# RazorClient/Stark-prover

Measured on AMD Instinct MI355X. Metric: FRI commit field-elems/sec at codeword 2^24; achieved HBM GB/s vs peak, higher is better.
Workload: dtype u32; 1 GPU; fri_commit codeword 2^24, blowup 8 (d=2^21), SHA-256 Merkle per layer, 21 rounds; codeword_log2=24, per_gpu_log2=24, blowup=8, field=p=3*2^30+1, parallelism=single GPU

## Files before the change

stark-prover_amd/csrc/fri_layer.hip:

```cpp
#include <cassert>
#include "fri_internal.hpp"
#include "sha256_fast.hpp"
#include "sha256_quad.hpp"

namespace fri {

#ifdef FRI_STAMPS
#define STAMP_WITH(on, i, fn)                                  \
    do {                                                       \
        if (on) t.st->stamps[t.k][(i)] = fn();                 \
    } while (0)
#else
#define STAMP_WITH(on, i, fn) do {} while (0)
#endif
#define STAMP(on, i) STAMP_WITH(on, i, __builtin_amdgcn_s_memrealtime)
#define STAMP_CLK(on, i) STAMP_WITH(on, i, __builtin_amdgcn_s_memtime)

#ifndef FRI_CHAIN_PRIO
#define FRI_CHAIN_PRIO 3
#endif
__device__ __forceinline__ void chain_prio() {
    if (FRI_CHAIN_PRIO > 0) __builtin_amdgcn_s_setprio(FRI_CHAIN_PRIO);
}

// ... 149 lines not shown
    coef_slice(t, w, G, red, 0, blockDim.x);
    lds_barrier();
    if (threadIdx.x == 0) coef_combine(t, w, red, blockDim.x / 64);
}

__device__ __forceinline__ void quad(const uint4& vals, uint32_t* lv0, uint32_t* lv1, size_t q ,
                                     Dg& out) {
    Dg a, b, c, d, n0, n1;
    hleaf(vals.x, a); hleaf(vals.y, b); hleaf(vals.z, c); hleaf(vals.w, d);
    dg_store(lv0 + 8 * (4 * q), a); dg_store(lv0 + 8 * (4 * q + 1), b);
    dg_store(lv0 + 8 * (4 * q + 2), c); dg_store(lv0 + 8 * (4 * q + 3), d);
    hnode(a, b, n0);
    hnode(c, d, n1);
    dg_store(lv1 + 8 * (2 * q), n0);
    dg_store(lv1 + 8 * (2 * q + 1), n1);
    hnode(n0, n1, out);
}

template <uint32_t TPB>
__device__ __forceinline__ void lds_two_levels(uint4* lds, const Dg& mine, uint32_t* lv2, uint32_t* lv3, uint32_t* lv4,
                                               size_t g2 ) {
    uint4* A = lds;
    uint4* B = lds + 2 * TPB;
    const uint32_t t = threadIdx.x;
    dg_store(lv2 + 8 * (g2 + t), mine);
    dg_lds_store(A + 2 * t, mine);
    lds_barrier();
    if (t < TPB / 2) {
        Dg l, r, o;
        dg_lds_load(A + 4 * t, l); dg_lds_load(A + 4 * t + 2, r);
        hnode(l, r, o);
        dg_lds_store(B + 2 * t, o);
        dg_store(lv3 + 8 * (g2 / 2 + t), o);
    }
    lds_barrier();
    if (t < TPB / 4) {
        Dg l, r, o;
        dg_lds_load(B + 4 * t, l); dg_lds_load(B + 4 * t + 2, r);
        hnode(l, r, o);
        dg_store(lv4 + 8 * (g2 / 4 + t), o);
    }
}

__device__ __forceinline__ bool gated_off(const LayerTask& t) {
    return t.gst && t.gidx >= 0 && !t.gst->active[t.gidx];
}

__device__ __forceinline__ uint32_t pair_beta(const LayerTask& t) { return t.gst->beta_mont[t.gidx]; }

template <bool FOLD, bool COMMIT, uint32_t TPB, bool PAIR = false>
__global__ __launch_bounds__(TPB) void k_layer_leaf(LayerTask t) {
    if (gated_off(t)) return;
    __shared__ uint4 lds[3 * TPB];
    __shared__ int32_t red[3 * (TPB / 64)];
    const uint32_t L = t.L;
    const size_t wg = PAIR ? (size_t)blockIdx.x + t.wg_base : (size_t)blockIdx.x;
    const size_t q = wg * TPB + threadIdx.x;
    uint4 v;
    if (FOLD) {
        const size_t half = (size_t)1 << L;
        const uint32_t beta_m = COMMIT ? t.st->beta_mont[t.k - 1] : (PAIR ? pair_beta(t) : t.beta_m);
        uint4 a = reinterpret_cast<const uint4*>(t.prev)[q];
        uint4 b = reinterpret_cast<const uint4*>(PAIR ? t.prev2 : t.prev + half)[q];
        uint4 x = reinterpret_cast<const uint4*>(t.xinv)[q];
        v.x = fold_one(a.x, b.x, x.x, beta_m); v.y = fold_one(a.y, b.y, x.y, beta_m);
        v.z = fold_one(a.z, b.z, x.z, beta_m); v.w = fold_one(a.w, b.w, x.w, beta_m);
        reinterpret_cast<uint4*>(t.values)[q] = v;
    } else {
        v = reinterpret_cast<const uint4*>(t.values)[q];
    }
    uint32_t* tr = t.tree;
    Dg top;
    quad(v, tr + 8 * level_offset(L, 0), tr + 8 * level_offset(L, 1), q, top);
    if (COMMIT) coef_task(t, blockIdx.x, gridDim.x, red);
    lds_two_levels<TPB>(lds, top, tr + 8 * level_offset(L, 2), tr + 8 * level_offset(L, 3),
                        tr + 8 * level_offset(L, 4), wg * TPB);
}

#ifndef WIDE_PAIR_MAX
#define WIDE_PAIR_MAX (1u << 16)
#endif

__host__ __device__ __forceinline__ uint32_t wide_levels(uint32_t L) { return L <= 8 + TOP_LOG ? 8u : 4u; }

template <bool FOLD, bool COMMIT, bool PAIR = false>
__global__ __launch_bounds__(256) void k_layer_leaf_wide(LayerTask t) {
    if (gated_off(t)) return;
    STAMP(COMMIT && blockIdx.x == 0 && threadIdx.x == 0, 60);
    __shared__ uint4 lds[2 * 256 + 2 * 128];
    __shared__ int32_t red[12];
    __shared__ SchedLds sl;
    sched_init(&sl);
    const uint32_t L = t.L;
    const size_t wg = PAIR ? (size_t)blockIdx.x + t.wg_base : (size_t)blockIdx.x;
    const size_t grid = PAIR ? (size_t)t.wg_total : (size_t)gridDim.x;
    const size_t i = wg * 256 + threadIdx.x;
    uint32_t v;
    if (FOLD) {
        const size_t half = (size_t)1 << L;
        const uint32_t beta_m = COMMIT ? t.st->beta_mont[t.k - 1] : (PAIR ? pair_beta(t) : t.beta_m);
        v = fold_one(t.prev[i], PAIR ? t.prev2[i] : t.prev[i + half], t.xinv[i], beta_m);
        t.values[i] = v;
    } else {
        v = t.values[i];
    }
    uint32_t* tr = t.tree;
    Dg d;
    cleaf(v, d);
    dg_store(tr + 8 * i, d);
    uint4* A = lds;
    uint4* B = lds + 2 * 256;
    dg_lds_store(A + 2 * threadIdx.x, d);
    lds_barrier();
    STAMP(COMMIT && blockIdx.x == 0 && threadIdx.x == 0, 61);
    uint32_t cnt = 256;
    const shaq::Role qr = shaq::role_of(threadIdx.x);
    if (grid * 128 < WIDE_PAIR_MAX) chain_prio();
    const uint32_t nlev = wide_levels(L);
#pragma unroll 1
    for (uint32_t j = 1; j <= nlev; j++) {
        cnt >>= 1;
        uint32_t* out = tr + 8 * (level_offset(L, j) + (wg << (8 - j)));
        if ((size_t)cnt * grid < WIDE_PAIR_MAX) {
            pair_level_s(A, B, out, threadIdx.x, cnt, qr, &sl, j);
        } else if (threadIdx.x < cnt) {
            Dg a, b, o;
            dg_lds_load(A + 4 * threadIdx.x, a);
            dg_lds_load(A + 4 * threadIdx.x + 2, b);
            hnode(a, b, o);
            dg_lds_store(B + 2 * threadIdx.x, o);
            dg_store(out + 8 * threadIdx.x, o);
        }
        if (COMMIT && j == 2 && threadIdx.x >= 128) coef_slice(t, blockIdx.x, gridDim.x, red, 128, 128);
        lds_barrier();
        uint4* tmp = A; A = B; B = tmp;
    }
    if (COMMIT && threadIdx.x == 128) coef_combine(t, blockIdx.x, red, 2);
    STAMP(COMMIT && blockIdx.x == 0 && threadIdx.x == 0, 62);
}

__device__ __forceinline__ void reduce_mx(const int32_t* in, int32_t* out, uint32_t w, uint32_t R) {
    if (threadIdx.x >= 64) return;
    Mx3 m;
    if (threadIdx.x < R) m.load(in, R * w + threadIdx.x);
    m.wave_max();
    if (threadIdx.x == 0) m.store(out, w);
}

__global__ __launch_bounds__(512) void k_tree_mid(uint32_t* tree, uint32_t L, uint32_t l, const DevState* st,
                                                  int gate, const int32_t* mx_in, int32_t* mx_out, uint32_t R) {
    if (st && gate >= 0 && !st->active[gate]) return;
    constexpr uint32_t NIN = 1024;
    __shared__ uint4 lds[NIN + NIN / 2];
    __shared__ SchedLds sl;
    sched_init(&sl);
    uint4* A = lds;
    uint4* B = lds + NIN;
    const uint32_t t = threadIdx.x;
    const size_t base = (size_t)blockIdx.x * NIN;
    const uint32_t* in = tree + 8 * level_offset(L, l);
    {
        Dg a, b, o;
        dg_load(in + 8 * (base + 2 * t), a);
        dg_load(in + 8 * (base + 2 * t + 1), b);
        if (mx_in) reduce_mx(mx_in, mx_out, blockIdx.x, R);
        hnode(a, b, o);
        dg_lds_store(A + 2 * t, o);
        dg_store(tree + 8 * (level_offset(L, l + 1) + (base >> 1) + t), o);
    }
    lds_barrier();
    const shaq::Role qr = shaq::role_of(t);
    uint32_t cnt = NIN / 2;
#pragma unroll 1
    for (uint32_t j = 2; j <= 4; j++) {
        cnt >>= 1;
        uint32_t* out = tree + 8 * (level_offset(L, l + j) + (base >> j));
        const bool narrow = (size_t)cnt * gridDim.x < WIDE_PAIR_MAX;
        if (narrow) {
            pair_level_s(A, B, out, t, cnt, qr, &sl, j);
        } else if (t < cnt) {
            Dg a, b, o;
            dg_lds_load(A + 4 * t, a);
            dg_lds_load(A + 4 * t + 2, b);
            hnode(a, b, o);
            dg_lds_store(B + 2 * t, o);
            dg_store(out + 8 * t, o);
        }
        lds_barrier();
        uint4* tmp = A; A = B; B = tmp;
    }
}

__global__ __launch_bounds__(256) void k_tree_mid8(uint32_t* tree, uint32_t L, uint32_t l, const DevState* st,
                                                   int gate, const int32_t* mx_in, int32_t* mx_out, uint32_t R) {
    if (st && gate >= 0 && !st->active[gate]) return;
    chain_prio();
    __shared__ uint4 lds[256 + 128];
    __shared__ SchedLds sl;
    sched_init(&sl);
    uint4* A = lds;
    uint4* B = lds + 256;
    const uint32_t t = threadIdx.x;
    const size_t base = (size_t)blockIdx.x * 256;
    const uint32_t* in = tree + 8 * level_offset(L, l);
    const shaq::Role qr = shaq::role_of(t);
    {
        const uint32_t q = t >> 1, half = (t & 1u) ^ 1u;
        Dg a, b;
        dg_load(in + 8 * (base + 2 * q), a);
        dg_load(in + 8 * (base + 2 * q + 1), b);
        if (mx_in) reduce_mx(mx_in, mx_out, blockIdx.x, R);
        uint32_t o[4];
        shaq::node(a.w, b.w, o, qr);
        const uint4 v = make_uint4(o[0], o[1], o[2], o[3]);
        A[2 * q + half] = v;
        reinterpret_cast<uint4*>(tree + 8 * (level_offset(L, l + 1) + (base >> 1) + q))[half] = v;
    }
    lds_barrier();
    uint32_t cnt = 128;
#pragma unroll 1
    for (uint32_t j = 2; j <= 8; j++) {
        cnt >>= 1;
        pair_level_s(A, B, tree + 8 * (level_offset(L, l + j) + (base >> j)), t, cnt, qr, &sl, j);
        lds_barrier();
        uint4* tmp = A; A = B; B = tmp;
    }
}

__device__ __forceinline__ void ktouch(const void* sym) {
    uint32_t a, b, c, d;
    asm volatile("s_nop 4\n\t"
                 "s_load_dword %0, %4, 0x0\n\ts_load_dword %1, %4, 0x40\n\t"
                 "s_load_dword %2, %4, 0x80\n\ts_load_dword %3, %4, 0xc0\n\t"
                 "s_waitcnt lgkmcnt(0)"
                 : "=&s"(a), "=&s"(b), "=&s"(c), "=&s"(d)
                 : "s"(sym)
                 : "memory");
}
__device__ __forceinline__ void kcache_touch_sha_tables() {
    ktouch(&shaf::KTAB[0]);
    ktouch(&shaf::PAD_KW_C.kw[0]);
    ktouch(&shaf::PAD_KW_1024.kw[0]);
    ktouch(&shaf::PAD_KW_1536.kw[0]);
}

__device__ __forceinline__ uint32_t hexch(uint32_t nib) { return nib < 10u ? 0x30u + nib : 0x57u + nib; }
__device__ __forceinline__ void hex2(uint32_t x, uint32_t& hi, uint32_t& lo) {
    hi = (hexch(x >> 28) << 24) | (hexch((x >> 24) & 15u) << 16) | (hexch((x >> 20) & 15u) << 8) | hexch((x >> 16) & 15u);
    lo = (hexch((x >> 12) & 15u) << 24) | (hexch((x >> 8) & 15u) << 16) | (hexch((x >> 4) & 15u) << 8) | hexch(x & 15u);
}
__device__ __forceinline__ uint32_t hexhex(uint32_t b) {
    const uint32_t x = ((b & 0xF0u) << 12) | (b & 0x0Fu);
    const uint32_t ge = ((x + 0x00060006u) >> 4) & 0x00010001u;
    return 0x33303330u + x + ge * 0x2F7u;
}

enum { CJ_REHASH = 0, CJ_MID = 2, CJ_ROOT = 3, CJ_FINAL = 6, CJ_END_ROUND = 6, CJ_END_FINAL = 8 };

__device__ __forceinline__ void chan_job(int j, uint32_t cs[8], uint32_t X[4], uint32_t has, const uint4* root_lds,
                                         uint32_t fv, const shaq::Role& R) {
    j = __builtin_amdgcn_readfirstlane(j);
    has = __builtin_amdgcn_readfirstlane(has);
    uint32_t w[16];
    const bool pad = (j == 1) || (j == 5);
    if (j == 0 || j == 2 || j == 6) {
#pragma unroll
        for (int i = 0; i < 8; i++) hex2(cs[i], w[2 * i], w[2 * i + 1]);
#pragma unroll
        for (int i = 0; i < 4; i++) X[i] = R.iv[i];
    } else if (j == 3 || j == 4) {
        const uint32_t b = (__lane_id() & 15u) + (j == 4 ? 16u : 0u);
        const uint32_t rw = reinterpret_cast<const uint32_t*>(root_lds)[b >> 2];
        const uint32_t hh = hexhex((rw >> (24 - 8 * (b & 3))) & 255u);
#pragma unroll
        for (int jj = 0; jj < 16; jj++) w[jj] = __builtin_amdgcn_readlane(hh, jj);
        if (j == 3 && !has) {
#pragma unroll
            for (int i = 0; i < 4; i++) X[i] = R.iv[i];
        }
    } else if (j == 7) {
#pragma unroll
        for (int i = 0; i < 16; i++) w[i] = 0u;
        w[0] = 0x30303030u; w[1] = 0x30303030u;
        hex2(fv, w[2], w[3]);
        w[4] = 0x80000000u;
        w[15] = 80u * 8u;
    }
    if (pad) shaq::compress_kw(X, j == 1 ? shaf::PAD_KW_C.kw : (has ? shaf::PAD_KW_1536.kw : shaf::PAD_KW_1024.kw), R);
    else shaq::compress(X, w, R);
    if (j == 1 || j == 5 || j == 7) {
#pragma unroll
        for (int i = 0; i < 4; i++) {
            const uint32_t o = shaq::swap01(X[i]);
            cs[i] = R.is_a ? X[i] : o;
            cs[4 + i] = R.is_a ? o : X[i];
        }
    }
}

constexpr uint32_t pow2_32k_mod_p(int k) {
    uint64_t r = 1;
    for (int j = 0; j < k; j++) r = (r << 32) % P;
    return (uint32_t)r;
}
__device__ __forceinline__ uint32_t chan_beta(const uint32_t s[8]) {
    constexpr uint32_t W[8] = {pow2_32k_mod_p(8), pow2_32k_mod_p(7), pow2_32k_mod_p(6), pow2_32k_mod_p(5),
                               pow2_32k_mod_p(4), pow2_32k_mod_p(3), pow2_32k_mod_p(2), pow2_32k_mod_p(1)};
    uint32_t t[8];
#pragma unroll
    for (int i = 0; i < 8; i++) t[i] = mmul(s[i] >= P ? s[i] - P : s[i], W[i]);
    return add(add(add(t[0], t[1]), add(t[2], t[3])), add(add(t[4], t[5]), add(t[6], t[7])));
}


template <typename Value>
__device__ __forceinline__ void leaf_loop(uint32_t N, uint32_t* tr, uint4* A, Value&& value) {
    for (uint32_t i = threadIdx.x; i < max(N, 64u); i += blockDim.x) {
        const uint32_t j = i & (N - 1);
        const bool real = i < N;
        const uint32_t v = value(j, real);
        Dg d;
        cleaf(v, d);
        if (real) {
            dg_store(tr + 8 * j, d);
            dg_lds_store(A + 2 * j, d);
        }
    }
}

__device__ __forceinline__ void level_step(const LayerTask& t, bool stamps, uint32_t it, const uint4* A, uint4* B,
                                           uint32_t* out, uint32_t cnt, const shaq::Role& R, SchedLds* sl,
                                           uint32_t ord) {
    const uint32_t tid = threadIdx.x;
    if (cnt <= 128) {
        STAMP_CLK(stamps && it < 18 && tid == 0, 24 + 2 * it);
        pair_level_s(A, B, out, tid, cnt, R, sl, ord);
        STAMP_CLK(stamps && it < 18 && tid == 0, 25 + 2 * it);
        return;
    }
#pragma unroll 1
    for (uint32_t q = tid; q < cnt; q += blockDim.x) {
        Dg a, b, o;
        dg_lds_load(A + 4 * q, a);
        dg_lds_load(A + 4 * q + 2, b);
#ifdef FRI_STAMPS
        if (stamps && it < 18 && q == 0) asm volatile("s_waitcnt lgkmcnt(0)" ::: "memory");
#endif
        STAMP_CLK(stamps && it < 18 && q == 0, 24 + 2 * it);
        cnode(a, b, o);
        STAMP_CLK(stamps && it < 18 && q == 0, 25 + 2 * it);
        dg_lds_store(B + 2 * q, o);
        dg_store(out + 8 * q, o);
    }
}

__device__ __forceinline__ int chan_drain(const LayerTask& t, int job, int job_end, bool level, uint32_t cnt,
                                           uint32_t cs[8], uint32_t X[4], uint32_t has, const uint4* root_lds,
                                           uint32_t fv, const shaq::Role& R) {
    if (job >= job_end || (level && !(cnt <= 192 && job < CJ_ROOT))) return job;
    do {
        STAMP(threadIdx.x == 448 && job == CJ_ROOT, 14);
        STAMP(threadIdx.x == 448 && job == CJ_ROOT + 2, 13);
        chan_job(job, cs, X, has, root_lds, fv, R);
        STAMP(threadIdx.x == 448 && job >= CJ_ROOT && job <= CJ_ROOT + 2, 20 + job - CJ_ROOT);
        job++;
    } while (!level && job < job_end);
    return job;
}

struct RoundOut { uint32_t active, beta_m; };
__device__ __forceinline__ RoundOut layer_results(const LayerTask& t, const Degree& dg, const uint32_t cs[8],
                                                  uint32_t fv, uint32_t fbeta1, const uint4* root_lds) {
    DevState* st = t.st;
    const int k = t.k, deg = dg.deg;
    if (dg.noncanon) {
        st->active[k] = 0;
// ... 231 lines not shown
                    const uint32_t c = t.coef_in[j];
                    if (c) m.m0 = max(m.m0, (int)j);
                    if (c >= P) m.m1 = 0;
                }
            } else {
                const uint32_t len = (uint32_t)(prev_deg + 1), nlen = (len + 1) / 2;
                const bool in_lds = li > 0 && k >= 2;
                for (uint32_t j = tx; j < nlen; j += nthr) {
                    const uint32_t e = in_lds ? prev_c[2 * j] : t.coef_in[2 * j];
                    const uint32_t o = (2 * j + 1 < len) ? (in_lds ? prev_c[2 * j + 1] : t.coef_in[2 * j + 1]) : 0u;
                    const uint32_t v = add(e, mmul(o, beta_m));
                    cur_c[j] = v;
                    if (v) m.m0 = (int)j;
                    if (e) m.m1 = (int)j;
                    if (o) m.m2 = (int)j;
                }
            }
            mx3_wave_to_red(m, red, tx);
        };
        if (!coef_late) coef_fold(0, blockDim.x);
        if (li == 0 && !coef_late) prefetch_x(0, blockDim.x);
        lds_barrier();
        STAMP(tid == 0, 1);
        STAMP_CLK(tid == 0, 17);
        Degree dg{1, false};
        int job_end = CJ_END_ROUND;
        uint32_t fv = 0;
        auto settle = [&](uint32_t nw) {
            dg = degree_of(k, mx3_from_red(red, nw));
            job_end = dg.deg < 1 ? CJ_END_FINAL : CJ_END_ROUND;
            if (chan_wave && dg.deg == 0) fv = (k == 0) ? t.coef_in[0] : cur_c[0];
        };
        if (!coef_late) settle(8);
        int job = CJ_END_FINAL;
        if (chan_wave) job = !has ? CJ_ROOT : (pending ? CJ_REHASH : CJ_MID);
        const uint32_t total = nlev + 1;
        uint32_t cnt = N;
#pragma unroll 1
        for (uint32_t it = 0; it < total; it++) {
            const bool level = it < nlev;
            if (level) {
                cnt >>= 1;
                level_step(t, true, it, A, B, tr + 8 * level_offset(L, 1 + it), cnt, R, &sl, ord++);
            }
            if (chan_wave) job = chan_drain(t, job, job_end, level, cnt, cs, X, has, A, fv, R);
            if (coef_late && it == coef_it && tid >= 256 && tid < 384) coef_fold(256, 128);
            if (li == 0 && coef_late && it == coef_it && tid >= 384 && tid < 448) prefetch_x(384, 64);
            lds_barrier();
            if (coef_late && it == coef_it) settle(2);
            if (level) {
                uint4* tmp = A; A = B; B = tmp;
                STAMP(tid == 0 && it < 11, 2 + it);
                STAMP_CLK(tid == 0 && it + 1 == nlev, 18);
                STAMP(tid == 0 && it + 1 == nlev, 19);
            }
        }
        if (tid == 448) {
            const RoundOut r = layer_results(t, dg, cs, fv, s_fbeta[li], A);
            s_beta_m = r.beta_m;
            s_active = r.active;
            s_deg = dg.deg;
        }
        if (chan_wave) { has = 1; pending = 1; }
        lds_barrier();
        if (!s_active) break;
        beta_m = s_beta_m;
        prev_deg = s_deg;
    }
}

static LayerTask with_gate(const LayerTask& in) {
    LayerTask t = in;
    if (t.st) { t.gst = t.st; t.gidx = t.k > 0 ? t.k - 1 : -1; }
    return t;
}

#ifndef QUAD_TPB
#define QUAD_TPB 512
#endif
#ifndef QUAD_MIN_LOG
#define QUAD_MIN_LOG 19
#endif

template <typename KernelLaunch>
static void pair_parts(LayerTask t, uint32_t G, hipStream_t s, const std::function<void()>& after_part1,
                       KernelLaunch&& go) {
    t.wg_total = G;
    if (!after_part1) {
        t.wg_base = 0;
        go(t, G);
        return;
    }
    const uint32_t h = G / 2;
    t.wg_base = t.send_half ? h : 0u;
    go(t, h);
    after_part1();
    t.wg_base = t.send_half ? 0u : h;
    go(t, h);
}

void launch_layer(const LayerTask& tin, hipStream_t s, hipEvent_t ev_leaf_end, const std::function<void()>& after_leaf,
                  hipEvent_t ev_before_top, const std::function<void()>& after_part1) {
    const LayerTask t = with_gate(tin);
    const uint32_t L = t.L;
    const bool fold = t.prev != nullptr;
    const bool commit = t.st != nullptr;
    const bool pair = t.prev2 != nullptr;
    const int32_t* nomx = nullptr;
    static_assert(TAIL_LOG == TOP_LOG, "every commit layer the top could take from its leaves goes to launch_tail");
    if (L <= TOP_LOG) {
        assert(!fold && !commit);
        hipLaunchKernelGGL((k_tree_top<true, false>), dim3(1), dim3(512), 0, s, t, 0u, nomx, 1u);
        if (ev_leaf_end) hipEventRecord(ev_leaf_end, s);
        return;
    }
    uint32_t G, out_per_wg;
    if (L >= QUAD_MIN_LOG) {
        constexpr uint32_t TPB = QUAD_TPB;
        G = (uint32_t)(((size_t)1 << L) / (4 * TPB));
        out_per_wg = TPB / 4;
        if (pair) {
            pair_parts(t, G, s, after_part1, [&](const LayerTask& tp, uint32_t g) {
                hipLaunchKernelGGL((k_layer_leaf<true, false, TPB, true>), dim3(g), dim3(TPB), 0, s, tp);
            });
        } else if (fold) {
            if (commit) hipLaunchKernelGGL((k_layer_leaf<true, true, TPB>), dim3(G), dim3(TPB), 0, s, t);
            else hipLaunchKernelGGL((k_layer_leaf<true, false, TPB>), dim3(G), dim3(TPB), 0, s, t);
        } else {
            if (commit) hipLaunchKernelGGL((k_layer_leaf<false, true, TPB>), dim3(G), dim3(TPB), 0, s, t);
            else hipLaunchKernelGGL((k_layer_leaf<false, false, TPB>), dim3(G), dim3(TPB), 0, s, t);
        }
    } else {
        G = 1u << (L - 8);
        out_per_wg = 256u >> wide_levels(L);
        if (pair) {
            pair_parts(t, G, s, after_part1, [&](const LayerTask& tp, uint32_t g) {
                hipLaunchKernelGGL((k_layer_leaf_wide<true, false, true>), dim3(g), dim3(256), 0, s, tp);
            });
        } else if (fold) {
            if (commit) hipLaunchKernelGGL((k_layer_leaf_wide<true, true>), dim3(G), dim3(256), 0, s, t);
            else hipLaunchKernelGGL((k_layer_leaf_wide<true, false>), dim3(G), dim3(256), 0, s, t);
        } else {
            if (commit) hipLaunchKernelGGL((k_layer_leaf_wide<false, true>), dim3(G), dim3(256), 0, s, t);
            else hipLaunchKernelGGL((k_layer_leaf_wide<false, false>), dim3(G), dim3(256), 0, s, t);
        }
    }
    if (ev_leaf_end) hipEventRecord(ev_leaf_end, s);
    if (after_leaf) after_leaf();
    const int gate = t.gidx;
    const int32_t* mx = commit ? t.wgmax : nullptr;
    size_t mx_off = 3 * (size_t)G;
    uint32_t l = L >= QUAD_MIN_LOG ? 4u : wide_levels(L);
    while (L - l > TOP_LOG) {
        const size_t nodes = (size_t)1 << (L - l);
        const bool eight = nodes < ((size_t)1 << 18);
        assert(!eight || L - l >= 8 + 6);
        const uint32_t nin = eight ? 256u : 1024u;
        const uint32_t grid = (uint32_t)(nodes / nin);
        const uint32_t R = nin / out_per_wg;
        int32_t* mx_out = commit ? t.wgmax + mx_off : nullptr;
        if (eight)
            hipLaunchKernelGGL(k_tree_mid8, dim3(grid), dim3(256), 0, s, t.tree, L, l, t.gst, gate, mx, mx_out, R);
        else
            hipLaunchKernelGGL(k_tree_mid, dim3(grid), dim3(512), 0, s, t.tree, L, l, t.gst, gate, mx, mx_out, R);
        if (commit) { mx = mx_out; mx_off += 3 * (size_t)grid; }
        G = grid;
        out_per_wg = eight ? 1u : nin / 16;
        l += eight ? 8u : 4u;
    }
    if (ev_before_top) hipStreamWaitEvent(s, ev_before_top, 0);
    if (commit) hipLaunchKernelGGL((k_tree_top<false, true>), dim3(1), dim3(512), 0, s, t, l, mx, G);
    else if (t.shard) hipLaunchKernelGGL((k_tree_top<false, false, true>), dim3(1), dim3(512), 0, s, t, l, nomx, G);
    else hipLaunchKernelGGL((k_tree_top<false, false>), dim3(1), dim3(512), 0, s, t, l, nomx, G);
}

void launch_tail(const LayerTask* ts, uint32_t n, hipStream_t s) {
    TailTask tt{};
    tt.n = n;
    for (uint32_t i = 0; i < n; i++) tt.t[i] = ts[i];
    tt.t[0] = with_gate(ts[0]);
    if (ts[0].prev) hipLaunchKernelGGL((k_tree_tail<true>), dim3(1), dim3(512), 0, s, tt);
    else hipLaunchKernelGGL((k_tree_tail<false>), dim3(1), dim3(512), 0, s, tt);
}

__global__ __launch_bounds__(256) void k_coef(LayerTask t) {
    if (gated_off(t)) return;
    __shared__ int32_t red[12];
    coef_task(t, blockIdx.x, gridDim.x, red);
}

void launch_coef(const LayerTask& tin, uint32_t G, hipStream_t s) {
    const LayerTask t = with_gate(tin);
    hipLaunchKernelGGL(k_coef, dim3(G), dim3(256), 0, s, t);
}

void launch_top(const LayerTask& tin, uint32_t l, const int32_t* mx, uint32_t G, hipStream_t s) {
    const LayerTask t = with_gate(tin);
    if (t.shard) hipLaunchKernelGGL((k_tree_top<false, true, true>), dim3(1), dim3(512), 0, s, t, l, mx, G);
    else hipLaunchKernelGGL((k_tree_top<false, true>), dim3(1), dim3(512), 0, s, t, l, mx, G);
}

}
```

stark-prover_amd/csrc/sha256_quad.hpp:

```cpp
#pragma once
#include <stdint.h>
#include "sha256_fast.hpp"

namespace fri {
namespace shaq {

constexpr int SWAP01 = 1 | (0 << 2) | (3 << 4) | (2 << 6);

__device__ __forceinline__ uint32_t swap01(uint32_t v) {
    return (uint32_t)__builtin_amdgcn_update_dpp(0, (int)v, SWAP01, 0xF, 0xF, true);
}
__device__ __forceinline__ uint32_t rot(uint32_t x, uint32_t n) { return __builtin_amdgcn_alignbit(x, x, n); }
#define bop(a, b, c, tt) __builtin_amdgcn_bitop3_b32((a), (b), (c), (tt))

struct Role {
    uint32_t r1, r2, r3;
    uint32_t m;
    uint32_t me;
    uint32_t q1, q2, q3;
    uint32_t is_a;
    uint32_t iv[4];
};

__device__ __forceinline__ Role role_of(uint32_t lane) {
    Role r{};
    const uint32_t IV[8] = {0x6a09e667u, 0xbb67ae85u, 0x3c6ef372u, 0xa54ff53au,
                            0x510e527fu, 0x9b05688cu, 0x1f83d9abu, 0x5be0cd19u};
    if ((lane & 1u) == 0) {
        r.r1 = 6; r.r2 = 11; r.r3 = 25; r.m = 0u; r.me = ~0u;
        r.q1 = 17; r.q2 = 19; r.q3 = 10; r.is_a = 0u;
        for (int i = 0; i < 4; i++) r.iv[i] = IV[4 + i];
    } else {
        r.r1 = 2; r.r2 = 13; r.r3 = 22; r.m = ~0u; r.me = 0u;
        r.q1 = 7; r.q2 = 18; r.q3 = 3; r.is_a = ~0u;
        for (int i = 0; i < 4; i++) r.iv[i] = IV[i];
    }
    return r;
}

#define SHAQ_R(kw)                                                                   \
    {                                                                                \
        const uint32_t _S = bop(rot(x0, R.r1), rot(x0, R.r2), rot(x0, R.r3), 0x96);  \
        const uint32_t _sel = bop(x0, x1, R.m, 0x2D);        \
        const uint32_t _F = bop(_sel, x2, x1, 0xCA);              \
        const uint32_t _hk = (x3 + (kw)) & R.me;                                     \
        const uint32_t _V = _S + _F + _hk;                                           \
        const uint32_t _Z = bop(R.me, _V, x3, 0xCA);                \
        const uint32_t _n = _V + swap01(_Z);                                         \
        x3 = x2; x2 = x1; x1 = x0; x0 = _n;                                          \
    }

#define SHAQ_W(i)                                                                            \
    {                                                                                        \
        const uint32_t _x = bop(R.is_a, w[((i) + 1) & 15], w[((i) + 14) & 15], 0xCA);        \
        const uint32_t _s = bop(rot(_x, R.q1), rot(_x, R.q2), _x >> R.q3, 0x96);             \
        w[i] = w[i] + w[((i) + 9) & 15] + _s + swap01(_s);                                   \
    }

__device__ __forceinline__ void compress(uint32_t st[4], uint32_t w[16], const Role& R) {
    uint32_t x0 = st[0], x1 = st[1], x2 = st[2], x3 = st[3];
#pragma unroll
    for (int i = 0; i < 16; i++) SHAQ_R(w[i] + shaf::KTAB[i]);
#pragma unroll 1
    for (int r = 1; r < 4; r++) {
#pragma unroll
        for (int i = 0; i < 16; i++) {
            SHAQ_W(i);
            SHAQ_R(w[i] + shaf::KTAB[16 * r + i]);
        }
    }
    st[0] += x0; st[1] += x1; st[2] += x2; st[3] += x3;
}
__device__ __forceinline__ void compress_kw(uint32_t st[4], const uint32_t* kw, const Role& R) {
    uint32_t x0 = st[0], x1 = st[1], x2 = st[2], x3 = st[3];
#pragma unroll 1
    for (int r = 0; r < 4; r++) {
#pragma unroll
        for (int i = 0; i < 16; i++) SHAQ_R(kw[16 * r + i]);
    }
    st[0] += x0; st[1] += x1; st[2] += x2; st[3] += x3;
}
__device__ __forceinline__ void produce(uint32_t w[16], uint32_t* wk, uint32_t* flag, uint32_t base, bool store,
                                        bool flag_lane, const Role& R) {
#pragma unroll 1
    for (int b = 0; b < 3; b++) {
#pragma unroll
        for (int i = 0; i < 16; i++) SHAQ_W(i);
        if (store) {
            uint4* o = reinterpret_cast<uint4*>(wk + 16 * b);
#pragma unroll
            for (int j = 0; j < 4; j++)
                o[j] = make_uint4(w[4 * j] + shaf::KTAB[16 * (b + 1) + 4 * j],
                                  w[4 * j + 1] + shaf::KTAB[16 * (b + 1) + 4 * j + 1],
                                  w[4 * j + 2] + shaf::KTAB[16 * (b + 1) + 4 * j + 2],
                                  w[4 * j + 3] + shaf::KTAB[16 * (b + 1) + 4 * j + 3]);
        }
        if (flag_lane) __hip_atomic_store(flag, base + b + 1, __ATOMIC_RELEASE, __HIP_MEMORY_SCOPE_WORKGROUP);
    }
}

__device__ __forceinline__ void node_ext(const uint32_t l[8], const uint32_t r[8], uint32_t out[4], const Role& R,
                                         const uint32_t* wk, const uint32_t* flag, uint32_t base) {
    uint32_t x0 = R.iv[0], x1 = R.iv[1], x2 = R.iv[2], x3 = R.iv[3];
#pragma unroll
    for (int i = 0; i < 8; i++) SHAQ_R(l[i] + shaf::KTAB[i]);
#pragma unroll
    for (int i = 0; i < 8; i++) SHAQ_R(r[i] + shaf::KTAB[8 + i]);
#pragma unroll 1
    for (int b = 0; b < 3; b++) {
        while (__hip_atomic_load(flag, __ATOMIC_ACQUIRE, __HIP_MEMORY_SCOPE_WORKGROUP) < base + b + 1) {}
        const uint4* q = reinterpret_cast<const uint4*>(wk + 16 * b);
        const uint4 q0 = q[0], q1 = q[1], q2 = q[2], q3 = q[3];
        SHAQ_R(q0.x); SHAQ_R(q0.y); SHAQ_R(q0.z); SHAQ_R(q0.w);
        SHAQ_R(q1.x); SHAQ_R(q1.y); SHAQ_R(q1.z); SHAQ_R(q1.w);
        SHAQ_R(q2.x); SHAQ_R(q2.y); SHAQ_R(q2.z); SHAQ_R(q2.w);
        SHAQ_R(q3.x); SHAQ_R(q3.y); SHAQ_R(q3.z); SHAQ_R(q3.w);
    }
    out[0] = R.iv[0] + x0; out[1] = R.iv[1] + x1; out[2] = R.iv[2] + x2; out[3] = R.iv[3] + x3;
    compress_kw(out, shaf::PAD_KW_C.kw, R);
}

#undef SHAQ_R
#undef SHAQ_W
#undef bop

__device__ __forceinline__ void node(const uint32_t l[8], const uint32_t r[8], uint32_t out[4], const Role& R) {
    uint32_t w[16];
#pragma unroll
    for (int i = 0; i < 8; i++) { w[i] = l[i]; w[8 + i] = r[i]; }
#pragma unroll
    for (int i = 0; i < 4; i++) out[i] = R.iv[i];
    compress(out, w, R);
    compress_kw(out, shaf::PAD_KW_C.kw, R);
}

}
}
```

Before: 3.649 billion field-elems/s.

## Add register-climb tree kernel collapsing mid Merkle levels into one launch

Adds a k_tree_climb kernel for subtrees of 2^18..2^20 nodes. Each thread hashes N consecutive nodes up in registers, then the block reduces through LDS for nine more levels, so a whole run of levels down to 256 outputs finishes in a single launch. This replaces several k_tree_mid/k_tree_mid8 launches and cuts launch count and intermediate round trips per layer. k_tree_mid drops its narrow quad-scheduled path. The cost is higher register pressure and serial per-thread hashing in the climb phase, which could lower occupancy.

```diff
diff --git a/stark-prover_amd/csrc/fri_layer.hip b/stark-prover_amd/csrc/fri_layer.hip
--- a/stark-prover_amd/csrc/fri_layer.hip
+++ b/stark-prover_amd/csrc/fri_layer.hip
@@ -325,8 +325,6 @@
     if (st && gate >= 0 && !st->active[gate]) return;
     constexpr uint32_t NIN = 1024;
     __shared__ uint4 lds[NIN + NIN / 2];
-    __shared__ SchedLds sl;
-    sched_init(&sl);
     uint4* A = lds;
     uint4* B = lds + NIN;
     const uint32_t t = threadIdx.x;
@@ -342,16 +340,12 @@
         dg_store(tree + 8 * (level_offset(L, l + 1) + (base >> 1) + t), o);
     }
     lds_barrier();
-    const shaq::Role qr = shaq::role_of(t);
     uint32_t cnt = NIN / 2;
 #pragma unroll 1
     for (uint32_t j = 2; j <= 4; j++) {
         cnt >>= 1;
         uint32_t* out = tree + 8 * (level_offset(L, l + j) + (base >> j));
-        const bool narrow = (size_t)cnt * gridDim.x < WIDE_PAIR_MAX;
-        if (narrow) {
-            pair_level_s(A, B, out, t, cnt, qr, &sl, j);
-        } else if (t < cnt) {
+        if (t < cnt) {
             Dg a, b, o;
             dg_lds_load(A + 4 * t, a);
             dg_lds_load(A + 4 * t + 2, b);
@@ -395,6 +389,85 @@
     for (uint32_t j = 2; j <= 8; j++) {
         cnt >>= 1;
         pair_level_s(A, B, tree + 8 * (level_offset(L, l + j) + (base >> j)), t, cnt, qr, &sl, j);
+        lds_barrier();
+        uint4* tmp = A; A = B; B = tmp;
+    }
+}
+
+template <uint32_t M>
+__device__ __forceinline__ void pair_up(Dg (&x)[M], Dg (&y)[M / 2]) {
+#pragma unroll 1
+    for (uint32_t i = 0; i < M / 2; i++) {
+        Dg o;
+        hnode(x[0], x[1], o);
+#pragma unroll
+        for (uint32_t k = 0; k + 2 < M; k++) x[k] = x[k + 2];
+#pragma unroll
+        for (uint32_t k = 0; k + 1 < M / 2; k++) y[k] = y[k + 1];
+        y[M / 2 - 1] = o;
+    }
+}
+template <uint32_t M>
+__device__ __forceinline__ void climb_regs(Dg (&x)[M], uint32_t* tree, uint32_t L, uint32_t lv, size_t g, Dg& root) {
+    Dg y[M / 2] = {};
+    pair_up<M>(x, y);
+    if constexpr (M == 2) {
+        root = y[0];
+    } else {
+        uint32_t* out = tree + 8 * (level_offset(L, lv) + (g >> 1));
+#pragma unroll
+        for (uint32_t i = 0; i < M / 2; i++) dg_store(out + 8 * i, y[i]);
+        climb_regs<M / 2>(y, tree, L, lv + 1, g >> 1, root);
+    }
+}
+
+template <uint32_t N>
+__global__ __launch_bounds__(512) void k_tree_climb(uint32_t* tree, uint32_t L, uint32_t l, const DevState* st,
+                                                    int gate, const int32_t* mx_in, int32_t* mx_out, uint32_t R) {
+    static_assert(N == 2 || N == 4 || N == 8, "2^18 .. 2^20 inputs over 256 x 512 threads");
+    if (st && gate >= 0 && !st->active[gate]) return;
+    constexpr uint32_t LOGN = N == 8 ? 3 : N == 4 ? 2 : 1;
+    __shared__ uint4 lds[2 * 512 + 2 * 256];
+    __shared__ SchedLds sl;
+    sched_init(&sl);
+    uint4* A = lds;
+    uint4* B = lds + 2 * 512;
+    const uint32_t t = threadIdx.x;
+    const size_t base = (size_t)blockIdx.x * (512 * N);
+    const size_t g = base + (size_t)N * t;
+    Dg top;
+    {
+        const uint32_t* in = tree + 8 * (level_offset(L, l) + g);
+        Dg x[N];
+#pragma unroll
+        for (uint32_t i = 0; i < N; i++) dg_load(in + 8 * i, x[i]);
+        if (mx_in) reduce_mx(mx_in, mx_out, blockIdx.x, R);
+        climb_regs<N>(x, tree, L, l + 1, g, top);
+    }
+    uint32_t lv = l + LOGN;
+    dg_store(tree + 8 * (level_offset(L, lv) + (base >> LOGN) + t), top);
+    dg_lds_store(A + 2 * t, top);
+    lds_barrier();
+    const shaq::Role qr = shaq::role_of(t);
+    uint32_t cnt = 512;
+    bool prio = false;
+#pragma unroll 1
+    for (uint32_t j = 1; j <= 9; j++) {
+        cnt >>= 1;
+        lv++;
+        uint32_t* out = tree + 8 * (level_offset(L, lv) + (base >> (lv - l)));
+        const bool narrow = (size_t)cnt * gridDim.x < WIDE_PAIR_MAX;
+        if (narrow) {
+            if (!prio) { chain_prio(); prio = true; }
+            pair_level_s(A, B, out, t, cnt, qr, &sl, j);
+        } else if (t < cnt) {
+            Dg a, b, o;
+            dg_lds_load(A + 4 * t, a);
+            dg_lds_load(A + 4 * t + 2, b);
+            hnode(a, b, o);
+            dg_lds_store(B + 2 * t, o);
+            dg_store(out + 8 * t, o);
+        }
         lds_barrier();
         uint4* tmp = A; A = B; B = tmp;
     }
@@ -932,21 +1005,30 @@
     size_t mx_off = 3 * (size_t)G;
     uint32_t l = L >= QUAD_MIN_LOG ? 4u : wide_levels(L);
     while (L - l > TOP_LOG) {
-        const size_t nodes = (size_t)1 << (L - l);
-        const bool eight = nodes < ((size_t)1 << 18);
-        assert(!eight || L - l >= 8 + 6);
-        const uint32_t nin = eight ? 256u : 1024u;
+        const uint32_t D = L - l;
+        const size_t nodes = (size_t)1 << D;
+        const bool climb = D >= 18 && D <= 20;
+        const bool eight = D < 18;
+        assert(!eight || D >= 8 + 6);
+        const uint32_t nin = climb ? 1u << (D - 8) : eight ? 256u : 1024u;
         const uint32_t grid = (uint32_t)(nodes / nin);
         const uint32_t R = nin / out_per_wg;
+        assert(R <= 64);
         int32_t* mx_out = commit ? t.wgmax + mx_off : nullptr;
-        if (eight)
+        if (climb && D == 20)
+            hipLaunchKernelGGL(k_tree_climb<8>, dim3(grid), dim3(512), 0, s, t.tree, L, l, t.gst, gate, mx, mx_out, R);
+        else if (climb && D == 19)
+            hipLaunchKernelGGL(k_tree_climb<4>, dim3(grid), dim3(512), 0, s, t.tree, L, l, t.gst, gate, mx, mx_out, R);
+        else if (climb)
+            hipLaunchKernelGGL(k_tree_climb<2>, dim3(grid), dim3(512), 0, s, t.tree, L, l, t.gst, gate, mx, mx_out, R);
+        else if (eight)
             hipLaunchKernelGGL(k_tree_mid8, dim3(grid), dim3(256), 0, s, t.tree, L, l, t.gst, gate, mx, mx_out, R);
         else
             hipLaunchKernelGGL(k_tree_mid, dim3(grid), dim3(512), 0, s, t.tree, L, l, t.gst, gate, mx, mx_out, R);
         if (commit) { mx = mx_out; mx_off += 3 * (size_t)grid; }
         G = grid;
-        out_per_wg = eight ? 1u : nin / 16;
-        l += eight ? 8u : 4u;
+        out_per_wg = climb || eight ? 1u : nin / 16;
+        l += climb ? D - 8 : eight ? 8u : 4u;
     }
     if (ev_before_top) hipStreamWaitEvent(s, ev_before_top, 0);
     if (commit) hipLaunchKernelGGL((k_tree_top<false, true>), dim3(1), dim3(512), 0, s, t, l, mx, G);
```

After: 3.639 billion field-elems/s. About the same (-0.3%).

## Hand-schedule quad SHA-256 rounds and message schedule in inline GCN assembly

Applied to the files above, without the earlier changes.

Replaces the compiler-generated SHA-256 round and message-schedule code in node_ext, produce and compress_kw with hand-written inline assembly. It uses v_add3, bitop3 and DPP-fused adds, software-pipelines the next round's h+K+W term, and streams the padding-block constants into hard-coded SGPRs s68-s99 with double-buffered s_load_dwordx16. The goal is fewer instructions and less dependency stall per round in the hash-bound Merkle kernel. It risks clobbering fixed SGPRs that may conflict with compiler allocation, depends on hand-placed s_nop/waitcnt hazards, and makes the code much more fragile.

```diff
diff --git a/stark-prover_amd/csrc/sha256_quad.hpp b/stark-prover_amd/csrc/sha256_quad.hpp
--- a/stark-prover_amd/csrc/sha256_quad.hpp
+++ b/stark-prover_amd/csrc/sha256_quad.hpp
@@ -57,6 +57,60 @@
         w[i] = w[i] + w[((i) + 9) & 15] + _s + swap01(_s);                                   \
     }
 
+#define SHAQ_RS(X0, X1, X2, X3, HK, HKN, NX, I)                                           \
+    "v_alignbit_b32 %[t1], %[" #X0 "], %[" #X0 "], %[r1]\n\t"                             \
+    "v_alignbit_b32 %[t2], %[" #X0 "], %[" #X0 "], %[r2]\n\t"                             \
+    "v_alignbit_b32 %[t3], %[" #X0 "], %[" #X0 "], %[r3]\n\t"                             \
+    "v_bitop3_b32 %[sel], %[" #X0 "], %[" #X1 "], %[m] bitop3:0x2d\n\t"                   \
+    "v_bitop3_b32 %[t1], %[t1], %[t2], %[t3] bitop3:0x96\n\t"                             \
+    "v_bitop3_b32 %[t2], %[sel], %[" #X2 "], %[" #X1 "] bitop3:0xca\n\t"                  \
+    "v_add3_u32 %[t1], %[t1], %[" #HK "], %[t2]\n\t"                                      \
+    "v_bitop3_b32 %[" #X3 "], %[me], %[t1], %[" #X3 "] bitop3:0xca\n\t"                   \
+    NX(HKN, X2, I)                                                                        \
+    "v_add_u32_dpp %[" #X3 "], %[" #X3 "], %[t1] quad_perm:[1,0,3,2] row_mask:0xf bank_mask:0xf bound_ctrl:1\n\t"
+#define SHAQ_NX_K(HKN, X2, I)                                                             \
+    "v_add_u32_e64 %[" #HKN "], %[k" #I "], %[" #X2 "]\n\t"                               \
+    "v_and_b32_e64 %[" #HKN "], %[" #HKN "], %[me]\n\t"
+#define SHAQ_NX_KR(HKN, X2, I)                                                            \
+    "v_add_u32_e64 %[" #HKN "], " I ", %[" #X2 "]\n\t"                                    \
+    "v_and_b32_e64 %[" #HKN "], %[" #HKN "], %[me]\n\t"
+#define SHAQ_NX_WK(HKN, X2, I)                                                            \
+    "v_add3_u32 %[" #HKN "], %[" #X2 "], %[w" #I "], %[k" #I "]\n\t"                      \
+    "v_and_b32_e64 %[" #HKN "], %[" #HKN "], %[me]\n\t"
+#define SHAQ_NX_NONE(HKN, X2, I) "s_nop 1\n\t"
+#define SHAQ_NX_TAIL(HKN, X2, I) I
+#define SHAQ_RS4(NX, L)                                                                   \
+    SHAQ_RS(a, b, c, d, ha, hb, NX, 1) SHAQ_RS(d, a, b, c, hb, ha, NX, 2)                 \
+    SHAQ_RS(c, d, a, b, ha, hb, NX, 3) SHAQ_RS(b, c, d, a, hb, ha, L, 4)
+#define SHAQ_RS8(NX, L)                                                                   \
+    SHAQ_RS(a, b, c, d, ha, hb, NX, 1) SHAQ_RS(d, a, b, c, hb, ha, NX, 2)                 \
+    SHAQ_RS(c, d, a, b, ha, hb, NX, 3) SHAQ_RS(b, c, d, a, hb, ha, NX, 4)                 \
+    SHAQ_RS(a, b, c, d, ha, hb, NX, 5) SHAQ_RS(d, a, b, c, hb, ha, NX, 6)                 \
+    SHAQ_RS(c, d, a, b, ha, hb, NX, 7) SHAQ_RS(b, c, d, a, hb, ha, L, 8)
+#define SHAQ_RS_STATE                                                                     \
+    [a] "+v"(x[0]), [b] "+v"(x[1]), [c] "+v"(x[2]), [d] "+v"(x[3]), [ha] "+v"(hk), [hb] "=&v"(hb_), \
+        [t1] "=&v"(t1_), [t2] "=&v"(t2_), [t3] "=&v"(t3_), [sel] "=&v"(sel_)
+#define SHAQ_RS_ROLE [r1] "v"(R.r1), [r2] "v"(R.r2), [r3] "v"(R.r3), [m] "v"(R.m), [me] "v"(R.me)
+#define SHAQ_K8(C) [k1] C(k[0]), [k2] C(k[1]), [k3] C(k[2]), [k4] C(k[3]), [k5] C(k[4]), [k6] C(k[5]), [k7] C(k[6]), [k8] C(k[7])
+
+template <bool LAST>
+__device__ __forceinline__ void rounds8_v(uint32_t x[4], uint32_t& hk, const uint32_t k[8], const Role& R) {
+    uint32_t hb_, t1_, t2_, t3_, sel_;
+#define SHAQ_C_V(v) "v"(v)
+    if (LAST) asm volatile(".p2align 3\n\t" SHAQ_RS8(SHAQ_NX_K, SHAQ_NX_NONE) : SHAQ_RS_STATE : SHAQ_K8(SHAQ_C_V), SHAQ_RS_ROLE);
+    else asm volatile(".p2align 3\n\t" SHAQ_RS8(SHAQ_NX_K, SHAQ_NX_K) : SHAQ_RS_STATE : SHAQ_K8(SHAQ_C_V), SHAQ_RS_ROLE);
+#undef SHAQ_C_V
+}
+template <bool LAST>
+__device__ __forceinline__ void rounds4_wk(uint32_t x[4], uint32_t& hk, const uint32_t w[4], const uint32_t k[4],
+                                           const Role& R) {
+    uint32_t hb_, t1_, t2_, t3_, sel_;
+#define SHAQ_WK4 [w1] "v"(w[0]), [w2] "v"(w[1]), [w3] "v"(w[2]), [w4] "v"(w[3]), [k1] "s"(k[0]), [k2] "s"(k[1]), [k3] "s"(k[2]), [k4] "s"(k[3])
+    if (LAST) asm volatile(".p2align 3\n\t" SHAQ_RS4(SHAQ_NX_WK, SHAQ_NX_NONE) : SHAQ_RS_STATE : SHAQ_WK4, SHAQ_RS_ROLE);
+    else asm volatile(".p2align 3\n\t" SHAQ_RS4(SHAQ_NX_WK, SHAQ_NX_WK) : SHAQ_RS_STATE : SHAQ_WK4, SHAQ_RS_ROLE);
+#undef SHAQ_WK4
+}
+
 __device__ __forceinline__ void compress(uint32_t st[4], uint32_t w[16], const Role& R) {
     uint32_t x0 = st[0], x1 = st[1], x2 = st[2], x3 = st[3];
 #pragma unroll
@@ -71,21 +125,87 @@
     }
     st[0] += x0; st[1] += x1; st[2] += x2; st[3] += x3;
 }
+__device__ __forceinline__ void compress_kw_plain(uint32_t st[4], const uint32_t* kw, const Role& R) {
+    uint32_t x0 = st[0], x1 = st[1], x2 = st[2], x3 = st[3];
+#pragma unroll 1
+    for (int r = 0; r < 4; r++) {
+#pragma unroll
+        for (int i = 0; i < 16; i++) SHAQ_R(kw[16 * r + i]);
+    }
+    st[0] += x0; st[1] += x1; st[2] += x2; st[3] += x3;
+}
+#define SHAQ_KGROUP(K0, K1, K2, K3, K4, K5, K6, K7, K8, K9, K10, K11, K12, K13, K14, K15, TAIL)  \
+    "v_add_u32_e64 %[ha], " K0 ", %[d]\n\t"                                                      \
+    "v_and_b32_e64 %[ha], %[ha], %[me]\n\t"                                                      \
+    SHAQ_RS(a, b, c, d, ha, hb, SHAQ_NX_KR, K1) SHAQ_RS(d, a, b, c, hb, ha, SHAQ_NX_KR, K2)      \
+    SHAQ_RS(c, d, a, b, ha, hb, SHAQ_NX_KR, K3) SHAQ_RS(b, c, d, a, hb, ha, SHAQ_NX_KR, K4)      \
+    SHAQ_RS(a, b, c, d, ha, hb, SHAQ_NX_KR, K5) SHAQ_RS(d, a, b, c, hb, ha, SHAQ_NX_KR, K6)      \
+    SHAQ_RS(c, d, a, b, ha, hb, SHAQ_NX_KR, K7) SHAQ_RS(b, c, d, a, hb, ha, SHAQ_NX_KR, K8)      \
+    SHAQ_RS(a, b, c, d, ha, hb, SHAQ_NX_KR, K9) SHAQ_RS(d, a, b, c, hb, ha, SHAQ_NX_KR, K10)     \
+    SHAQ_RS(c, d, a, b, ha, hb, SHAQ_NX_KR, K11) SHAQ_RS(b, c, d, a, hb, ha, SHAQ_NX_KR, K12)    \
+    SHAQ_RS(a, b, c, d, ha, hb, SHAQ_NX_KR, K13) SHAQ_RS(d, a, b, c, hb, ha, SHAQ_NX_KR, K14)    \
+    SHAQ_RS(c, d, a, b, ha, hb, SHAQ_NX_KR, K15) SHAQ_RS(b, c, d, a, hb, ha, SHAQ_NX_TAIL, TAIL)
+#define SHAQ_KGROUP_A(TAIL) SHAQ_KGROUP("s68", "s69", "s70", "s71", "s72", "s73", "s74", "s75", "s76", "s77", "s78", "s79", "s80", "s81", "s82", "s83", TAIL)
+#define SHAQ_KGROUP_B(TAIL) SHAQ_KGROUP("s84", "s85", "s86", "s87", "s88", "s89", "s90", "s91", "s92", "s93", "s94", "s95", "s96", "s97", "s98", "s99", TAIL)
 __device__ __forceinline__ void compress_kw(uint32_t st[4], const uint32_t* kw, const Role& R) {
-    uint32_t x0 = st[0], x1 = st[1], x2 = st[2], x3 = st[3];
-#pragma unroll 1
-    for (int r = 0; r < 4; r++) {
-#pragma unroll
-        for (int i = 0; i < 16; i++) SHAQ_R(kw[16 * r + i]);
-    }
-    st[0] += x0; st[1] += x1; st[2] += x2; st[3] += x3;
-}
+    uint32_t x[4] = {st[0], st[1], st[2], st[3]};
+    uint32_t hk, hb_, t1_, t2_, t3_, sel_;
+    asm volatile("s_load_dwordx16 s[68:83], %[kw], 0x0\n\t"
+                 "s_mov_b32 s64, 0\n\t"
+                 "s_waitcnt lgkmcnt(0)\n\t"
+                 "s_load_dwordx16 s[84:99], %[kw], 0x40\n\t"
+                 ".p2align 3\n"
+                 "1:\n\t"
+                 SHAQ_KGROUP_A("s_waitcnt lgkmcnt(0)\n\ts_load_dwordx16 s[68:83], %[kw], 0x80\n\ts_nop 0\n\t")
+                 SHAQ_KGROUP_B("s_waitcnt lgkmcnt(0)\n\ts_xor_b32 s64, s64, 1\n\ts_cbranch_scc0 2f\n\t"
+                               "s_load_dwordx16 s[84:99], %[kw], 0xc0\n"
+                               "2:\n\ts_nop 0\n\t")
+                 "s_cbranch_scc1 1b"
+                 : [a] "+v"(x[0]), [b] "+v"(x[1]), [c] "+v"(x[2]), [d] "+v"(x[3]), [ha] "=&v"(hk), [hb] "=&v"(hb_),
+                   [t1] "=&v"(t1_), [t2] "=&v"(t2_), [t3] "=&v"(t3_), [sel] "=&v"(sel_)
+                 : [kw] "s"(kw), SHAQ_RS_ROLE
+                 : "scc", "s64", "s68", "s69", "s70", "s71", "s72", "s73", "s74", "s75", "s76", "s77", "s78", "s79", "s80",
+                   "s81", "s82", "s83", "s84", "s85", "s86", "s87", "s88", "s89", "s90", "s91", "s92", "s93", "s94", "s95",
+                   "s96", "s97", "s98", "s99");
+    st[0] += x[0]; st[1] += x[1]; st[2] += x[2]; st[3] += x[3];
+}
+#define SHAQ_WS1(I1, I14) "v_bitop3_b32 %[sx], %[isa], %[w" #I1 "], %[w" #I14 "] bitop3:0xca\n\t"
+#define SHAQ_WS2(I, I9)                                                                   \
+    "v_alignbit_b32 %[t1], %[sx], %[sx], %[q1]\n\t"                                       \
+    "v_alignbit_b32 %[t2], %[sx], %[sx], %[q2]\n\t"                                       \
+    "v_lshrrev_b32_e64 %[t3], %[q3], %[sx]\n\t"                                           \
+    "v_bitop3_b32 %[ss], %[t1], %[t2], %[t3] bitop3:0x96\n\t"                             \
+    "v_add3_u32 %[w" #I "], %[w" #I "], %[w" #I9 "], %[ss]\n\t"
+#define SHAQ_WS3(I) \
+    "v_add_u32_dpp %[w" #I "], %[ss], %[w" #I "] quad_perm:[1,0,3,2] row_mask:0xf bank_mask:0xf bound_ctrl:1\n\t"
 __device__ __forceinline__ void produce(uint32_t w[16], uint32_t* wk, uint32_t* flag, uint32_t base, bool store,
                                         bool flag_lane, const Role& R) {
+    uint32_t sx_, ss_, t1_, t2_, t3_;
 #pragma unroll 1
     for (int b = 0; b < 3; b++) {
-#pragma unroll
-        for (int i = 0; i < 16; i++) SHAQ_W(i);
+        asm volatile(".p2align 3\n\t"
+                     SHAQ_WS1(1, 14) SHAQ_WS2(0, 9)
+                     SHAQ_WS1(2, 15) SHAQ_WS3(0) SHAQ_WS2(1, 10)
+                     SHAQ_WS1(3, 0) SHAQ_WS3(1) SHAQ_WS2(2, 11)
+                     SHAQ_WS1(4, 1) SHAQ_WS3(2) SHAQ_WS2(3, 12)
+                     SHAQ_WS1(5, 2) SHAQ_WS3(3) SHAQ_WS2(4, 13)
+                     SHAQ_WS1(6, 3) SHAQ_WS3(4) SHAQ_WS2(5, 14)
+                     SHAQ_WS1(7, 4) SHAQ_WS3(5) SHAQ_WS2(6, 15)
+                     SHAQ_WS1(8, 5) SHAQ_WS3(6) SHAQ_WS2(7, 0)
+                     SHAQ_WS1(9, 6) SHAQ_WS3(7) SHAQ_WS2(8, 1)
+                     SHAQ_WS1(10, 7) SHAQ_WS3(8) SHAQ_WS2(9, 2)
+                     SHAQ_WS1(11, 8) SHAQ_WS3(9) SHAQ_WS2(10, 3)
+                     SHAQ_WS1(12, 9) SHAQ_WS3(10) SHAQ_WS2(11, 4)
+                     SHAQ_WS1(13, 10) SHAQ_WS3(11) SHAQ_WS2(12, 5)
+                     SHAQ_WS1(14, 11) SHAQ_WS3(12) SHAQ_WS2(13, 6)
+                     SHAQ_WS1(15, 12) SHAQ_WS3(13) SHAQ_WS2(14, 7)
+                     SHAQ_WS1(0, 13) SHAQ_WS3(14) SHAQ_WS2(15, 8)
+                     "s_nop 0\n\t" SHAQ_WS3(15)
+                     : [w0] "+v"(w[0]), [w1] "+v"(w[1]), [w2] "+v"(w[2]), [w3] "+v"(w[3]), [w4] "+v"(w[4]), [w5] "+v"(w[5]),
+                       [w6] "+v"(w[6]), [w7] "+v"(w[7]), [w8] "+v"(w[8]), [w9] "+v"(w[9]), [w10] "+v"(w[10]),
+                       [w11] "+v"(w[11]), [w12] "+v"(w[12]), [w13] "+v"(w[13]), [w14] "+v"(w[14]), [w15] "+v"(w[15]),
+                       [sx] "=&v"(sx_), [ss] "=&v"(ss_), [t1] "=&v"(t1_), [t2] "=&v"(t2_), [t3] "=&v"(t3_)
+                     : [q1] "v"(R.q1), [q2] "v"(R.q2), [q3] "v"(R.q3), [isa] "v"(R.is_a));
         if (store) {
             uint4* o = reinterpret_cast<uint4*>(wk + 16 * b);
 #pragma unroll
@@ -101,27 +221,52 @@
 
 __device__ __forceinline__ void node_ext(const uint32_t l[8], const uint32_t r[8], uint32_t out[4], const Role& R,
                                          const uint32_t* wk, const uint32_t* flag, uint32_t base) {
-    uint32_t x0 = R.iv[0], x1 = R.iv[1], x2 = R.iv[2], x3 = R.iv[3];
-#pragma unroll
-    for (int i = 0; i < 8; i++) SHAQ_R(l[i] + shaf::KTAB[i]);
-#pragma unroll
-    for (int i = 0; i < 8; i++) SHAQ_R(r[i] + shaf::KTAB[8 + i]);
+    uint32_t x[4] = {R.iv[0], R.iv[1], R.iv[2], R.iv[3]};
+    uint32_t w[16], k[16];
+#pragma unroll
+    for (int i = 0; i < 8; i++) { w[i] = l[i]; w[8 + i] = r[i]; }
+#pragma unroll
+    for (int i = 0; i < 16; i++) k[i] = shaf::KTAB[i];
+    uint32_t hk = (x[3] + w[0] + k[0]) & R.me;
+    rounds4_wk<false>(x, hk, w + 1, k + 1, R);
+    rounds4_wk<false>(x, hk, w + 5, k + 5, R);
+    rounds4_wk<false>(x, hk, w + 9, k + 9, R);
+    const uint32_t wl[4] = {w[13], w[14], w[15], w[15]}, kl[4] = {k[13], k[14], k[15], k[15]};
+    rounds4_wk<true>(x, hk, wl, kl, R);
 #pragma unroll 1
     for (int b = 0; b < 3; b++) {
         while (__hip_atomic_load(flag, __ATOMIC_ACQUIRE, __HIP_MEMORY_SCOPE_WORKGROUP) < base + b + 1) {}
         const uint4* q = reinterpret_cast<const uint4*>(wk + 16 * b);
         const uint4 q0 = q[0], q1 = q[1], q2 = q[2], q3 = q[3];
-        SHAQ_R(q0.x); SHAQ_R(q0.y); SHAQ_R(q0.z); SHAQ_R(q0.w);
-        SHAQ_R(q1.x); SHAQ_R(q1.y); SHAQ_R(q1.z); SHAQ_R(q1.w);
-        SHAQ_R(q2.x); SHAQ_R(q2.y); SHAQ_R(q2.z); SHAQ_R(q2.w);
-        SHAQ_R(q3.x); SHAQ_R(q3.y); SHAQ_R(q3.z); SHAQ_R(q3.w);
-    }
-    out[0] = R.iv[0] + x0; out[1] = R.iv[1] + x1; out[2] = R.iv[2] + x2; out[3] = R.iv[3] + x3;
+        const uint32_t qa[8] = {q0.y, q0.z, q0.w, q1.x, q1.y, q1.z, q1.w, q2.x};
+        const uint32_t qb[8] = {q2.y, q2.z, q2.w, q3.x, q3.y, q3.z, q3.w, q3.w};
+        hk = (x[3] + q0.x) & R.me;
+        rounds8_v<false>(x, hk, qa, R);
+        rounds8_v<true>(x, hk, qb, R);
+    }
+    out[0] = R.iv[0] + x[0]; out[1] = R.iv[1] + x[1]; out[2] = R.iv[2] + x[2]; out[3] = R.iv[3] + x[3];
     compress_kw(out, shaf::PAD_KW_C.kw, R);
 }
 
 #undef SHAQ_R
 #undef SHAQ_W
+#undef SHAQ_RS
+#undef SHAQ_NX_K
+#undef SHAQ_NX_WK
+#undef SHAQ_NX_NONE
+#undef SHAQ_RS4
+#undef SHAQ_RS8
+#undef SHAQ_RS_STATE
+#undef SHAQ_RS_ROLE
+#undef SHAQ_K8
+#undef SHAQ_WS1
+#undef SHAQ_WS2
+#undef SHAQ_WS3
+#undef SHAQ_NX_KR
+#undef SHAQ_NX_TAIL
+#undef SHAQ_KGROUP
+#undef SHAQ_KGROUP_A
+#undef SHAQ_KGROUP_B
 #undef bop
 
 __device__ __forceinline__ void node(const uint32_t l[8], const uint32_t r[8], uint32_t out[4], const Role& R) {
```

Measured after the change: 3.665 billion field-elems/s before, 3.697 billion field-elems/s after, median of 6. About the same (+0.9%).
